# ChainSafe/lumenos

Measured on AMD Instinct MI355X. Metric: prove_eval_seconds_16384x4096, lower is better.
Workload: dtype u64; 1 GPU; Encode+Commit+InnerProduct(r,b)+QueryCols 16384x4096 LogN=14 L=12 K=2 rhoInv=2 queries=309; parallelism=1 GPU: the whole job resident in HBM

## Files before the change

lumenos_amd/csrc/lm_keyswitch.hip:

```cpp
#include <cstdlib>
#include <cstring>

#include "lm_ks_dev.h"

__host__ __device__ __forceinline__ size_t ks_ext_at(uint32_t b, uint32_t d, uint32_t t, uint32_t B, uint32_t beta) {
    return ((size_t)t * B + b) * beta + d;
}
__host__ __device__ __forceinline__ size_t ks_u_at(uint32_t pw, uint32_t t, uint32_t B, uint32_t L, uint32_t K) {
    return t < L ? (size_t)t * 2 * B + pw : (size_t)L * 2 * B + (size_t)pw * K + (t - L);
}
__host__ __device__ __forceinline__ size_t ks_key_at(uint32_t d, uint32_t w, uint32_t t, uint32_t beta) {
    return ((size_t)t * beta + d) * 2 + w;
}

static uint32_t ks_batch(const lumen_ctx *ctx) { return ctx->tune.ks_batch; }

__device__ __forceinline__ void mul128(u64 a, u64 b, u64 &lo, u64 &hi) {
    const u32 a0 = (u32)a, a1 = (u32)(a >> 32), b0 = (u32)b, b1 = (u32)(b >> 32);
    const u64 p0 = (u64)a0 * b0;
    const u64 p1 = lm_keep((u64)a0 * b1 + (p0 >> 32));
    const u64 p2 = lm_keep((u64)a1 * b0 + (u32)p1);
    hi = (u64)a1 * b1 + (p1 >> 32) + (p2 >> 32);
    lo = (p2 << 32) | (u32)p0;
}
// ... 67 lines not shown
        return;
    }
    const uint32_t d = blockIdx.x / B, b = blockIdx.x % B;
    const uint32_t l0 = 2 * d, l1 = l0 + 1;
    const u64 *c1 = acc + ((size_t)b * 2 + 1) * L * N;
    u64 *o0 = coef + ((size_t)b * L + l0) * N;
    const lm_qc q0 = lm_make_qc(mods.m[l0]);
    const tw_t s0 = yscale.t[l0];
    {
        const u64 *p = c1 + (size_t)l0 * N;
        auto ld = [&](uint32_t i0, u64 *v, int count) { lm_load_run(p, i0, v, count); };
        auto st = [&](uint32_t i, u64 v) { o0[i] = lm_shoup_cs(v, s0, q0.q, q0.nq); };
        lm_ntt_inverse<LOGN>(sm, tw_all + (size_t)l0 * N, q0, tid, nthreads, ld, st);
    }
    __syncthreads();
    {
        const lm_qc q1 = lm_make_qc(mods.m[l1]);
        const tw_t s1 = yscale.t[l1];
        const u64 *p = c1 + (size_t)l1 * N;
        u64 Ml, Mh;
        mul128(q0.q, q1.q, Ml, Mh);
        auto uni = [](u64 x) {
            return (u64)(uint32_t)__builtin_amdgcn_readfirstlane((int)(uint32_t)x) |
                   (u64)(uint32_t)__builtin_amdgcn_readfirstlane((int)(uint32_t)(x >> 32)) << 32;
        };
        const u128 M = ((u128)uni(Mh) << 64) | uni(Ml);
        auto ld = [&](uint32_t i0, u64 *v, int count) { lm_load_run(p, i0, v, count); };
        constexpr int R_LAST = lm_pass_r(LOGN, 0), LOG_T0 = LOGN - R_LAST;
        constexpr int PF = (1 << R_LAST) * 5 / 8;
        struct pack_t {
            u64 *o0;
            const lm_qc &q0, &q1;
            tw_t s1;
            u128 M;
            u64 y0[PF];
            __device__ __forceinline__ void pre(uint32_t w) {
#pragma unroll
                for (int k = 0; k < PF; k++) y0[k] = o0[w + ((uint32_t)k << LOG_T0)];
            }
            __device__ __forceinline__ void operator()(uint32_t i, u64 v, int k) {
                const u64 y1 = lm_shoup_cs(v, s1, q1.q, q1.nq);
                uint32_t j = i;
                asm volatile("" : "+v"(j));
                const u64 a = k < PF ? y0[k < PF ? k : 0] : o0[j];
                u64 hi, lo;
                pack_pair(a, y1, q0.q, q1.q, M, hi, lo);
                o0[j] = hi, o0[j + N] = lo;
                if (k >= PF && (k & 1)) asm volatile("" ::: "memory");
            }
        } st{o0, q0, q1, s1, M, {}};
        uint32_t tid1 = tid;
        asm volatile("" : "+v"(tid1));
        lm_ntt_inverse<LOGN>(sm, tw_all + (size_t)l1 * N, q1, tid1, nthreads, ld, st);
    }
}

struct pt_consts_t {
    u64 c[LM_MAX_LIMBS];
};
__global__ void k_pt_prepare(const u64 *__restrict__ pt, u64 *__restrict__ ptM, uint32_t logN, uint32_t nl,
                             lm_mods mods, pt_consts_t pc) {
    const size_t total = (size_t)nl << logN;
    for (size_t i = (size_t)blockIdx.x * blockDim.x + threadIdx.x; i < total; i += (size_t)gridDim.x * blockDim.x) {
        const uint32_t limb = (uint32_t)(i >> logN);
        u64 lo, hi;
        mul128(pt[i], pc.c[limb], lo, hi);
        ptM[i] = lm_mont_reduce(lo, hi, mods.m[limb].q, mods.m[limb].qneg);
    }
}
__global__ void k_mul_plain(const u64 *__restrict__ ct, u64 *__restrict__ out, const u64 *__restrict__ ptM,
                            size_t words, uint32_t logN, uint32_t nl, lm_mods mods) {
    const size_t stride = (size_t)gridDim.x * blockDim.x;
    const size_t N = (size_t)1 << logN;
    for (size_t i = (size_t)blockIdx.x * blockDim.x + threadIdx.x; i < words; i += stride) {
        const uint32_t limb = (uint32_t)((i >> logN) % nl);
        const size_t k = i & (N - 1);
        u64 lo, hi;
        mul128(ct[i], ptM[(size_t)limb * N + k], lo, hi);
        out[i] = lm_mont_reduce(lo, hi, mods.m[limb].q, mods.m[limb].qneg);
    }
}

template <int LOGN>
__global__ __launch_bounds__(lm_max_threads(LOGN)) void k_modup_ntt(const u64 *__restrict__ coef, const u64 *__restrict__ acc,
                                                    u64 *__restrict__ ext, const bx_t *__restrict__ bx,
                                                    uint32_t B, uint32_t L, uint32_t K, uint32_t beta,
                                                    const uint32_t *__restrict__ work, lm_mods mods,
                                                    const tw_t *__restrict__ tw_all) {
    extern __shared__ __attribute__((aligned(16))) u64 sm[];
    constexpr uint32_t N = 1u << LOGN;
    const uint32_t tid = threadIdx.x, nthreads = blockDim.x, LK = L + K;
    const uint32_t wk = work[blockIdx.x];
    const uint32_t b = wk & 0xFFFF, d = (wk >> 16) & 0xFF, t = wk >> 24;
    const bx_t c = bx[d * LK + t];
    u64 *o = ext + ks_ext_at(b, d, t, B, beta) * N;
    const lm_qc qc = lm_make_qc(mods.m[t]);
    const u64 *s0 = coef + ((size_t)b * L + d * K) * N;
    const u64 *s1 = c.ns == 2 ? s0 + N : s0;
    auto ld = [&](uint32_t i) { return bx_apply(c, s0[i], s1[i], qc); };
    lm_lds_runs st{sm};
    auto after = [&](uint32_t, uint32_t) {
        lm_linear_out<LOGN>(sm, tid, [&](uint32_t j, u64 v0, u64 v1) {
            ulonglong2 y;
            y.x = v0, y.y = v1;
            *reinterpret_cast<ulonglong2 *>(o + j) = y;
        });
    };
    lm_ntt_forward<LOGN>(sm, tw_all + (size_t)t * N, qc, tid, nthreads, ld, st, after);
}

#ifndef LM_MAC_COLS
#define LM_MAC_COLS 4
#endif
#ifndef LM_MAC_VEC
#define LM_MAC_VEC 1
#endif
#ifndef LM_MAC_PREFETCH
#define LM_MAC_PREFETCH 1
#endif
template <int VEC>
struct mac_vec;
template <>
struct mac_vec<1> {
    u64 v[1];
    static __device__ __forceinline__ mac_vec load(const u64 *p) { return mac_vec{{*p}}; }
    static __device__ __forceinline__ mac_vec load_once(const u64 *p) { return mac_vec{{__builtin_nontemporal_load(p)}}; }
    __device__ __forceinline__ void store(u64 *p) const { *p = v[0]; }
};
template <>
struct mac_vec<2> {
    u64 v[2];
    static __device__ __forceinline__ mac_vec load(const u64 *p) {
        const ulonglong2 a = *reinterpret_cast<const ulonglong2 *>(p);
        return mac_vec{{a.x, a.y}};
    }
    static __device__ __forceinline__ mac_vec load_once(const u64 *p) {
        return mac_vec{{__builtin_nontemporal_load(p), __builtin_nontemporal_load(p + 1)}};
    }
    __device__ __forceinline__ void store(u64 *p) const {
        ulonglong2 a;
        a.x = v[0], a.y = v[1];
        *reinterpret_cast<ulonglong2 *>(p) = a;
    }
};
struct mac_acc {
    u64 a0, a1, a3;
    u32 c0, c1;
    __device__ __forceinline__ void clear() { a0 = a1 = a3 = 0, c0 = c1 = 0; }
    __device__ __forceinline__ void value(u64 &lo, u64 &hi) const {
        lo = a0 + (a1 << 32);
        hi = a3 + c0 + (a1 >> 32) + ((u64)c1 << 32) + (lo < a0 ? 1 : 0);
    }
};
__device__ __forceinline__ void mac2(mac_acc &p, mac_acc &q, u64 x, u64 k0, u64 k1) {
    const u32 x0 = (u32)x, x1 = (u32)(x >> 32);
#if LM_ASM_SHOUP
    asm("v_mad_u64_u32 %[pa0], s[98:99], %[x0], %[k00], %[pa0]\n\t"
        "v_mad_u64_u32 %[qa0], s[90:91], %[x0], %[k10], %[qa0]\n\t"
        "v_mad_u64_u32 %[pa1], s[94:95], %[x0], %[k01], %[pa1]\n\t"
        "v_addc_co_u32_e64 %[pc0], s[96:97], %[pc0], 0, s[98:99]\n\t"
        "v_mad_u64_u32 %[qa1], s[92:93], %[x0], %[k11], %[qa1]\n\t"
        "v_addc_co_u32_e64 %[qc0], s[96:97], %[qc0], 0, s[90:91]\n\t"
        "v_mad_u64_u32 %[pa3], s[96:97], %[x1], %[k01], %[pa3]\n\t"
        "v_addc_co_u32_e64 %[pc1], s[96:97], %[pc1], 0, s[94:95]\n\t"
        "v_mad_u64_u32 %[pa1], s[98:99], %[x1], %[k00], %[pa1]\n\t"
        "v_addc_co_u32_e64 %[qc1], s[96:97], %[qc1], 0, s[92:93]\n\t"
        "v_mad_u64_u32 %[qa1], s[90:91], %[x1], %[k10], %[qa1]\n\t"
        "v_mad_u64_u32 %[qa3], s[96:97], %[x1], %[k11], %[qa3]\n\t"
        "v_addc_co_u32_e64 %[pc1], s[96:97], %[pc1], 0, s[98:99]\n\t"
        "v_addc_co_u32_e64 %[qc1], s[96:97], %[qc1], 0, s[90:91]"
        : [pa0] "+v"(p.a0), [pa1] "+v"(p.a1), [pa3] "+v"(p.a3), [pc0] "+v"(p.c0), [pc1] "+v"(p.c1),
          [qa0] "+v"(q.a0), [qa1] "+v"(q.a1), [qa3] "+v"(q.a3), [qc0] "+v"(q.c0), [qc1] "+v"(q.c1)
        : [x0] "v"(x0), [x1] "v"(x1), [k00] "v"((u32)k0), [k01] "v"((u32)(k0 >> 32)), [k10] "v"((u32)k1),
          [k11] "v"((u32)(k1 >> 32))
        : "s92", "s93", "s94", "s95", "s96", "s97", "s98", "s99", "s90", "s91");
#else
    auto one = [&](mac_acc &r, u64 k) {
        const u32 k0w = (u32)k, k1w = (u32)(k >> 32);
        u64 t = r.a0 + (u64)x0 * k0w;
        r.c0 += t < r.a0, r.a0 = t;
        t = r.a1 + (u64)x0 * k1w;
        r.c1 += t < r.a1, r.a1 = t;
        t = r.a1 + (u64)x1 * k0w;
        r.c1 += t < r.a1, r.a1 = t;
        r.a3 += (u64)x1 * k1w;
    };
    one(p, k0);
    one(q, k1);
#endif
}

// ... 372 lines not shown
    static const uint32_t v = [&] {
        hipDeviceProp_t prop;
        int per_cu = 0;
        if (hipGetDeviceProperties(&prop, ctx->device) != hipSuccess) return 256u;
        (void)hipFuncSetAttribute(reinterpret_cast<const void *>(&k_intt_pack<LOGN>),
                                  hipFuncAttributeMaxDynamicSharedMemorySize, 160 * 1024);
        if (hipOccupancyMaxActiveBlocksPerMultiprocessor(&per_cu, k_intt_pack<LOGN>, lm_nthreads(LOGN),
                                                         lm_lds_for(1u << LOGN)) != hipSuccess || per_cu < 1) {
            per_cu = (int)std::max<size_t>(1, std::min<size_t>(160 * 1024 / lm_lds_for(1u << LOGN), 2048 / lm_nthreads(LOGN)));
        }
        (void)hipGetLastError();
        if (ctx->tune.debug)
            fprintf(stderr, "[lumenos_hip] k_intt_pack<%d>: %d workgroup(s) per CU, %d CUs\n", LOGN, per_cu,
                    prop.multiProcessorCount);
        return (uint32_t)prop.multiProcessorCount * (uint32_t)per_cu;
    }();
    return v;
}
static uint32_t ks_fused_digits(lumen_ctx *ctx, uint32_t B, uint32_t L) {
    const long forced = ctx->tune.ks_fused_digits;
    const uint32_t pairs = L / 2;
    if (forced >= 0) return std::min<uint32_t>((uint32_t)forced, pairs);
    uint32_t slots = 0;
    switch (ctx->logN) {
#define LM_CASE(n) \
    case n: slots = intt_pack_slots<n>(ctx); break;
        LM_FOR_EACH_LOGN(LM_CASE)
#undef LM_CASE
    default: return 0;
    }
    for (uint32_t nf = pairs; nf >= 1; nf--)
        if (((uint64_t)B * nf) % slots == 0) return nf;
    return 0;
}

struct LaneGuard {
    lumen_ctx *ctx;
    hipStream_t saved;
    LaneGuard(lumen_ctx *c, int lane) : ctx(c), saved(c->stream) {
        if (lane) ctx->stream = ctx->stream2;
    }
    ~LaneGuard() { ctx->stream = saved; }
};

int rotate_accumulate(lumen_ctx *ctx, const u64 *acc, u64 *acc_out, uint32_t B, const lm_galois_key &gk,
                      KsTables *tb, const KsScratch &s) {
    const uint32_t N = ctx->N, L = ctx->L, K = ctx->K, LK = L + K, beta = tb->beta;
    const size_t lds = lm_fwd_lds(ctx->logN);
    const uint32_t threads = lm_fwd_threads(ctx->logN);
    const uint32_t nf = K == 2 ? ks_fused_digits(ctx, B, L) : 0;
    if (nf) {
        const size_t lds_i = lm_inv_lds(ctx->logN);
        const uint32_t grid = B * nf + B * (L - 2 * nf);
        lm_prof_scope ps(ctx, "ks_intt_c1", (uint64_t)B * L);
        switch (ctx->logN) {
#define LM_CASE(n)                                                                                              \
    case n:                                                                                                     \
        LM_LDS_ATTR(ctx, k_intt_pack<n>, lds_i);                                                                \
        hipLaunchKernelGGL(k_intt_pack<n>, dim3(grid), dim3(lm_inv_threads(ctx->logN)), lds_i, ctx->stream, acc, \
                           s.coef, B, L, nf, ctx->mods, tb->yscale, ctx->d_tw_inv);                             \
        break;
            LM_FOR_EACH_LOGN(LM_CASE)
#undef LM_CASE
        default:
            return lm_fail(ctx, "ring degree 2^%u has no kernel instantiation", ctx->logN);
        }
        LM_HIP(ctx, hipGetLastError());
    } else {
        if (int rc = lm_launch_ntt_strided(ctx, acc + (size_t)L * N, (size_t)2 * L * N, s.coef, (size_t)L * N, B,
                                           lm_map_q(L), true, "ks_intt_c1", &tb->yscale))
            return rc;
    }
    if (K == 2 && nf < beta) {
        lm_prof_scope ps(ctx, "ks_pack_v", (uint64_t)B);
        hipLaunchKernelGGL(k_pack_v, dim3(2048), dim3(256), 0, ctx->stream, s.coef + (size_t)2 * nf * N, (size_t)L * N,
                           B, beta - nf, K, 2 * nf, L - 2 * nf, ctx->logN, ctx->mods);
        LM_HIP(ctx, hipGetLastError());
    }
    {
        const uint64_t nb = (uint64_t)B * tb->pairs.size();
        const uint32_t *work = nullptr;
        if (int rc = modup_work_list(ctx, tb, B, &work)) return rc;
        lm_prof_scope ps(ctx, "ks_modup_ntt", nb);
        switch (ctx->logN) {
#define LM_CASE(n)                                                                                            \
    case n:                                                                                                   \
        LM_LDS_ATTR(ctx, k_modup_ntt<n>, lds);               \
        hipLaunchKernelGGL(k_modup_ntt<n>, dim3((uint32_t)nb), dim3(threads), lds, ctx->stream, s.coef, acc,  \
                           s.ext, tb->d_bx, B, L, K, beta, work, ctx->mods, ctx->d_tw_fwd);                   \
        break;
            LM_FOR_EACH_LOGN(LM_CASE)
#undef LM_CASE
        default:
            return lm_fail(ctx, "ring degree 2^%u has no kernel instantiation", ctx->logN);
        }
        LM_HIP(ctx, hipGetLastError());
    }
    {
        lm_prof_scope ps(ctx, "ks_mac", (uint64_t)B);
        dim3 grid(((N / LM_MAC_VEC + 255) / 256) * LK * ((B + LM_MAC_COLS - 1) / LM_MAC_COLS));
        hipLaunchKernelGGL(k_ks_mac, grid, dim3(256), 0, ctx->stream, s.ext, acc, gk.d_key, s.u, B, L, K, beta,
                           ctx->logN, ctx->mods);
        LM_HIP(ctx, hipGetLastError());
    }
    {
        lm_modmap mp;
        mp.period = K;
        for (uint32_t i = 0; i < LM_MAX_LIMBS; i++) mp.idx[i] = (uint8_t)(L + (i < K ? i : 0));
        u64 *up = s.u + ks_u_at(0, L, B, L, K) * N;
        const size_t pstride = (size_t)K * N;
        if (int rc = lm_launch_ntt_strided(ctx, up, pstride, up, pstride, B * 2, mp, true, "ks_intt_p", &tb->yscale))
            return rc;
        if (K == 2) {
            lm_prof_scope ps(ctx, "ks_pack_v", (uint64_t)B);
            hipLaunchKernelGGL(k_pack_v, dim3(2048), dim3(256), 0, ctx->stream, up, pstride, B * 2, 1u, K, L, K,
                               ctx->logN, ctx->mods);
            LM_HIP(ctx, hipGetLastError());
        }
    }
    {
        const uint32_t *work_down = nullptr;
        if (int rc = moddown_work_list(ctx, tb, B, &work_down)) return rc;
        lm_prof_scope ps(ctx, "ks_moddown_ntt", (uint64_t)B * 2 * L);
        switch (ctx->logN) {
#define LM_CASE(n)                                                                                            \
    case n:                                                                                                   \
        LM_LDS_ATTR(ctx, k_moddown_ntt<n>, lds);               \
        hipLaunchKernelGGL(k_moddown_ntt<n>, dim3(B * 2 * L), dim3(threads), lds, ctx->stream, s.u, acc,      \
                           acc_out, tb->d_bxp, tb->d_pinv, gk.d_index, gk.d_inv_index, work_down, B, L, K, ctx->mods, \
                           ctx->d_tw_fwd);                                                                    \
        break;
            LM_FOR_EACH_LOGN(LM_CASE)
#undef LM_CASE
        default:
            return lm_fail(ctx, "ring degree 2^%u has no kernel instantiation", ctx->logN);
        }
        LM_HIP(ctx, hipGetLastError());
    }
    return 0;
}

int get_scratch(lumen_ctx *ctx, uint32_t B, KsTables *tb, KsScratch *s, int lane = 0, u64 **group_acc = nullptr,
                size_t group_acc_bytes = 0) {
    const size_t N = ctx->N, L = ctx->L, LK = ctx->L + ctx->K, beta = tb->beta;
    const char *names[2][5] = {{"ks_coef", "ks_ext", "ks_u", "ks_acc2", "ks_acc"}, {"ks_coef_b", "ks_ext_b", "ks_u_b", "ks_acc2_b", "ks_acc"}};
    const int NB = group_acc ? 5 : 4;
    const size_t bytes[5] = {(size_t)B * L * N * 8, (size_t)B * beta * LK * N * 8, (size_t)B * 2 * LK * N * 8, (size_t)B * 2 * L * N * 8,
                             std::max(group_acc_bytes, (size_t)B * 2 * L * N * 8)};
    u64 *dummy = nullptr;
    u64 **slot[5] = {&s->coef, &s->ext, &s->u, &s->acc2, group_acc ? group_acc : &dummy};
    bool have = true;
    for (int c = 0; c < NB; c++) {
        auto it = ctx->scratch.find(names[lane][c]);
        have = have && it != ctx->scratch.end() && it->second.first && it->second.second >= bytes[c];
    }
    lm_galois_key gk;
    {
        LM_SHARED_LOCK(ctx);
        if (!ctx->gkeys.empty()) gk = ctx->gkeys.begin()->second;
    }
    const uint32_t Kc = ctx->tune.ks_placement;
    auto plain = [&]() -> int {
        bool ok = true;
        for (int c = 0; c < NB; c++) ok = (*slot[c] = (u64 *)lm_scratch(ctx, names[lane][c], bytes[c])) != nullptr && ok;
        return ok ? 0 : 1;
    };
    if (have || Kc < 2 || bytes[1] < ((size_t)64 << 20) || !gk.d_key) return plain();
    std::vector<void *> cand[5];
    bool fixed[5] = {false, false, false, false, false};
    for (int c = 0; c < NB; c++) {
        auto it = ctx->scratch.find(names[lane][c]);
// ... 401 lines not shown
```

lumenos_amd/csrc/lm_ntt.hip:

```cpp
#include "lm_ntt_dev.h"

template <int LOGN, bool INV>
__global__ __launch_bounds__(lm_max_threads(LOGN)) void k_limb_ntt(const u64 *src, size_t src_poly_stride, u64 *dst,
                                                   size_t dst_poly_stride, uint32_t npoly, lm_modmap map,
                                                   lm_mods mods, lm_ninv_t ninv,
                                                   const tw_t *__restrict__ tw_all) {
    extern __shared__ __attribute__((aligned(16))) u64 sm[];
    constexpr uint32_t N = 1u << LOGN;
    const uint32_t tid = threadIdx.x, nthreads = blockDim.x;
    const uint32_t limb = blockIdx.x / npoly, poly = blockIdx.x % npoly;
    const uint32_t mi = map.idx[limb];
    const lm_qc c = lm_make_qc(mods.m[mi]);
    const u64 *p = src + (size_t)poly * src_poly_stride + (size_t)limb * N;
    u64 *o = dst + (size_t)poly * dst_poly_stride + (size_t)limb * N;
    const tw_t *tw = tw_all + (size_t)mi * N;
    if (INV) {
        const tw_t ni = ninv.t[mi];
        auto st = [&](uint32_t i, u64 v) { o[i] = lm_shoup_cs(v, ni, c.q, c.nq); };
        auto ld = [&](uint32_t i0, u64 *v, int count) { lm_load_run(p, i0, v, count); };
        lm_ntt_inverse<LOGN>(sm, tw, c, tid, nthreads, ld, st);
    } else {
        auto ld = [&](uint32_t i) { return p[i]; };
        auto st = [&](uint32_t i0, const u64 *v, int count) {
            u64 r[8];
#pragma unroll
            for (int k = 0; k < 8; k++)
                if (k < count) r[k] = lm_reduce_s(v[k], c.q, c.nq, c.qinv64);
            lm_store_run(o, i0, r, count);
        };
        lm_ntt_forward<LOGN>(sm, tw, c, tid, nthreads, ld, st);
    }
}

int lm_launch_ntt_subring(lumen_ctx *ctx, uint32_t logn, const tw_t *tw, tw_t ninv_scale, const u64 *src,
                          size_t src_poly_stride, u64 *dst, size_t dst_poly_stride, uint32_t npoly,
                          uint32_t mod_idx, bool inverse, const mod_t *explicit_mod) {
    if (!npoly) return 0;
    lm_modmap map = lm_map_q(1);
    map.idx[0] = 0;
    lm_mods mods = ctx->mods;
    mods.m[0] = explicit_mod ? *explicit_mod : ctx->mods.m[mod_idx];
    lm_ninv_t ninv = lm_ninv_of(ctx);
    ninv.t[0] = ninv_scale;
    const size_t lds = inverse ? lm_inv_lds(logn) : lm_fwd_lds(logn);
    const uint32_t threads = inverse ? lm_inv_threads(logn) : lm_fwd_threads(logn);
    const dim3 grid(npoly), block(threads);
#define LM_LAUNCH(n)                                                                                          \
    case n:                                                                                                   \
        if (inverse) {                                                                                        \
            LM_LDS_ATTR(ctx, (k_limb_ntt<n, true>), lds);                                                     \
            hipLaunchKernelGGL((k_limb_ntt<n, true>), grid, block, lds, ctx->stream, src, src_poly_stride,    \
                               dst, dst_poly_stride, npoly, map, mods, ninv, tw);                             \
        } else {                                                                                              \
            LM_LDS_ATTR(ctx, (k_limb_ntt<n, false>), lds);                                                    \
            hipLaunchKernelGGL((k_limb_ntt<n, false>), grid, block, lds, ctx->stream, src, src_poly_stride,   \
                               dst, dst_poly_stride, npoly, map, mods, ninv, tw);                             \
        }                                                                                                     \
        break;
    switch (logn) {
        LM_FOR_EACH_LOGN(LM_LAUNCH)
    default:
        return lm_fail(ctx, "ring degree 2^%u has no kernel instantiation", logn);
    }
#undef LM_LAUNCH
    LM_HIP(ctx, hipGetLastError());
    return 0;
}

int lm_launch_ntt_strided(lumen_ctx *ctx, const u64 *src, size_t src_poly_stride, u64 *dst,
                          size_t dst_poly_stride, uint32_t npoly, const lm_modmap &map, bool inverse,
                          const char *prof_name, const lm_ninv_t *inv_scale) {
    if (!npoly || !map.period) return 0;
    const uint32_t N = ctx->N;
    const lm_ninv_t ninv = inv_scale ? *inv_scale : lm_ninv_of(ctx);
    const size_t lds = inverse ? lm_inv_lds(ctx->logN) : lm_fwd_lds(ctx->logN);
    const uint32_t threads = inverse ? lm_inv_threads(ctx->logN) : lm_fwd_threads(ctx->logN);
    (void)N;
    const uint64_t nblocks64 = (uint64_t)npoly * map.period;
    LM_CHECK(ctx, nblocks64 < (1ull << 31), "NTT grid too large: %llu", (unsigned long long)nblocks64);
    lm_prof_scope ps(ctx, prof_name ? prof_name : (inverse ? "limb_intt" : "limb_ntt"), nblocks64);
    const dim3 grid((uint32_t)nblocks64), block(threads);
#define LM_LAUNCH(n)                                                                                          \
    case n:                                                                                                   \
        if (inverse) {                                                                                        \
            LM_LDS_ATTR(ctx, (k_limb_ntt<n, true>), lds);           \
            hipLaunchKernelGGL((k_limb_ntt<n, true>), grid, block, lds, ctx->stream, src, src_poly_stride,    \
                               dst, dst_poly_stride, npoly, map, ctx->mods, ninv, ctx->d_tw_inv);             \
        } else {                                                                                              \
            LM_LDS_ATTR(ctx, (k_limb_ntt<n, false>), lds);           \
            hipLaunchKernelGGL((k_limb_ntt<n, false>), grid, block, lds, ctx->stream, src, src_poly_stride,   \
                               dst, dst_poly_stride, npoly, map, ctx->mods, ninv, ctx->d_tw_fwd);             \
        }                                                                                                     \
        break;
    switch (ctx->logN) {
        LM_FOR_EACH_LOGN(LM_LAUNCH)
    default:
        return lm_fail(ctx, "ring degree 2^%u has no kernel instantiation", ctx->logN);
    }
#undef LM_LAUNCH
    LM_HIP(ctx, hipGetLastError());
    return 0;
}

int lm_launch_ntt(lumen_ctx *ctx, u64 *d, uint32_t npoly, const lm_modmap &map, bool inverse) {
    const size_t stride = (size_t)map.period * ctx->N;
    return lm_launch_ntt_strided(ctx, d, stride, d, stride, npoly, map, inverse, nullptr, nullptr);
}

extern "C" int lumen_set_ntt(lumen_ctx *ctx, lumen_set *set, int inverse) {
    LM_CHECK(nullptr, ctx && set, "lumen_set_ntt: NULL argument");
    LM_ENTER(ctx);
    LM_FULL_WIDTH(ctx, set, "lumen_set_ntt");
    return lm_launch_ntt(ctx, set->d, set->count * 2, lm_map_q(set->nl), inverse != 0);
}
```

lumenos_amd/csrc/lm_ntt_dev.h:

```cpp
#pragma once
#include <cstring>
#include <type_traits>
#include <utility>

#include "lm_common.h"

#define LM_PAD(i) ((i) + ((i) >> 3))
template <int LOG_STRIDE>
__device__ __forceinline__ uint32_t lm_pad_at(uint32_t base, uint32_t pbase, int k) {
    if constexpr (LOG_STRIDE >= 3)
        return pbase + (uint32_t)k * ((1u << LOG_STRIDE) + (1u << (LOG_STRIDE - 3)));
    else
        return LM_PAD(base + ((uint32_t)k << LOG_STRIDE));
}
#define LM_MAX_PASSES 8

struct lm_ninv_t {
    tw_t t[LM_MAX_LIMBS];
};

__host__ __device__ constexpr int lm_ilog2(int x) { return x <= 1 ? 0 : 1 + lm_ilog2(x >> 1); }
#ifndef LM_COEFS_PER_LANE
#define LM_COEFS_PER_LANE 16
#endif
// ... 389 lines not shown
        lm_fwd_first<LOGN, R, cross>(sm, tw, c, tid, ld);
    else if constexpr (P == NP - 1)
        lm_fwd_last<LOGN, R>(sm, tw, c, tid, st);
    else
        lm_fwd_mid<LOGN, R, S0>(sm, tw, c, tid);
    if constexpr (P + 1 < NP) {
        if constexpr (P == 0 && cross)
            __syncthreads();
        else
            lm_wave_sync();
        lm_fwd_rec<LOGN, P + 1, S0 + R>(sm, tw, c, tid, ld, st);
    }
}
template <int LOGN>
__host__ __device__ constexpr int lm_fwd_run() {
    return 1 << lm_pass_r(LOGN, lm_npasses(LOGN) - 1);
}
struct lm_no_after {
    __device__ __forceinline__ void operator()(uint32_t, uint32_t) const {}
};

#ifndef LM_TW_XPASS
#define LM_TW_XPASS 1
#endif
template <int LOGN, int R, int S0, bool UW>
__device__ __forceinline__ void lm_fwd_mid_item(u64 *s, const lm_twset<R, UW> &T, const lm_qc &c, uint32_t w) {
    constexpr uint32_t log_tl = LOGN - S0 - R;
    const uint32_t blk = w >> log_tl, off = w & ((1u << log_tl) - 1);
    const uint32_t base = (blk << (log_tl + R)) + off;
    u64 e[1 << R];
    const uint32_t pb = LM_PAD(base);
#pragma unroll
    for (int k = 0; k < (1 << R); k++) e[k] = s[lm_pad_at<log_tl>(base, pb, k)];
    lm_fwd_stages<R, UW>(e, T, c);
#pragma unroll
    for (int k = 0; k < (1 << R); k++) s[lm_pad_at<log_tl>(base, pb, k)] = e[k];
}
template <class Loader, class Storer>
__device__ __forceinline__ void lm_fwd14_xpass(u64 *sm, const tw_t *tw, const lm_qc &c, uint32_t tid, Loader &ld,
                                               Storer &st) {
    constexpr int LOGN = 14;
    static_assert(lm_npasses(LOGN) == 4 && lm_pass_r(LOGN, 0) == 4 && lm_pass_r(LOGN, 1) == 4 &&
                      lm_pass_r(LOGN, 2) == 3 && lm_pass_r(LOGN, 3) == 3,
                  "written for the pass plan 4 | 4 3 3");
    using D4 = lm_deal<LOGN, 4>;
    using D3 = lm_deal<LOGN, 3>;
    static_assert(D4::reps == 1 && D3::reps == 2, "one item in pass 1, two in passes 2 and 3");
    lm_fwd_first<LOGN, 4, true>(sm, tw, c, tid, ld);
    lm_twset<4, true> T1;
    T1.load(tw, 4, D4::local(tid, 0) >> (LOGN - 8));
    __syncthreads();
    lm_twset<3, false> A, B;
    A.load(tw, 8, D3::local(tid, 0) >> (LOGN - 11));
    B.load(tw, 8, D3::local(tid, 1) >> (LOGN - 11));
    lm_fwd_mid_item<LOGN, 4, 4, true>(sm, T1, c, D4::local(tid, 0));
    lm_wave_sync();
    lm_fwd_mid_item<LOGN, 3, 8, false>(sm, A, c, D3::local(tid, 0));
    A.load(tw, 11, D3::local(tid, 0));
    lm_fwd_mid_item<LOGN, 3, 8, false>(sm, B, c, D3::local(tid, 1));
    B.load(tw, 11, D3::local(tid, 1));
    lm_wave_sync();
#pragma unroll
    for (uint32_t m = 0; m < 2; m++) {
        const uint32_t base = D3::local(tid, m) << 3;
        u64 e[8];
#pragma unroll
        for (int k = 0; k < 8; k++) e[k] = sm[LM_PAD(base + k)];
        lm_fwd_stages<3, false>(e, m ? B : A, c);
        st(base, e, 8);
    }
}

template <int LOGN, bool XPASS = true, class Loader, class Storer, class After = lm_no_after>
__device__ __forceinline__ void lm_ntt_forward(u64 *sm, const tw_t *tw, const lm_qc &c, uint32_t tid, uint32_t,
                                               Loader &ld, Storer &st, After after = After()) {
    static_assert(lm_npasses(LOGN) >= 2, "a transform needs a loading and a storing pass");
    if constexpr (LOGN == 14 && XPASS && LM_TW_XPASS && LM_COEFS_PER_LANE == 16 && !lm_has_pre<Storer>::value)
        lm_fwd14_xpass(sm, tw, c, tid, ld, st);
    else
        lm_fwd_rec<LOGN, 0, 0>(sm, tw, c, tid, ld, st);
    after(0u, 1u << LOGN);
}

template <int LOGN, int R, class Loader>
__device__ __forceinline__ void lm_inv_first(u64 *s, const tw_t *tw, const lm_qc &c, uint32_t tid, Loader &ld) {
    using D = lm_deal<LOGN, R>;
    if (!D::valid(tid)) return;
#pragma unroll 1
    for (uint32_t m = 0; m < D::reps; m++) {
        const uint32_t w = D::local(tid, m);
        const uint32_t base = w << R;
        u64 e[1 << R];
        lm_inv_twset<R, false, true> T;
        T.load(tw, LOGN, 0, w);
        ld(base, e, 1 << R);
        lm_inv_stages<R, false, false, true>(e, T, c);
#pragma unroll
        for (int k = 0; k < (1 << R); k++) s[LM_PAD(base + k)] = e[k];
    }
}

#ifndef LM_INV_TW_PREFETCH
#define LM_INV_TW_PREFETCH 1
#endif
template <int LOGN, int R, int LT>
__device__ __forceinline__ void lm_inv_mid(u64 *s, const tw_t *tw, const lm_qc &c, uint32_t tid) {
    using D = lm_deal<LOGN, R>;
    if (!D::valid(tid)) return;
    constexpr bool UW = LT >= 6;
    lm_inv_twset<R, UW, false> T[2];
    T[0].load(tw, LOGN, LT, D::local(tid, 0) >> LT);
#pragma unroll
    for (uint32_t m = 0; m < D::reps; m++) {
        const uint32_t w = D::local(tid, m);
        const uint32_t blk = w >> LT, off = w & ((1u << LT) - 1);
        const uint32_t base = (blk << (LT + R)) + off;
        u64 e[1 << R];
        const uint32_t pb = LM_PAD(base);
#pragma unroll
        for (int k = 0; k < (1 << R); k++) e[k] = s[lm_pad_at<LT>(base, pb, k)];
        if (LM_INV_TW_PREFETCH && m + 1 < D::reps) T[(m + 1) & 1].load(tw, LOGN, LT, D::local(tid, m + 1) >> LT);
        if (!LM_INV_TW_PREFETCH && m) T[0].load(tw, LOGN, LT, blk);
        lm_inv_stages<R, UW, false, false>(e, T[LM_INV_TW_PREFETCH ? (m & 1) : 0], c);
#pragma unroll
        for (int k = 0; k < (1 << R); k++) s[lm_pad_at<LT>(base, pb, k)] = e[k];
    }
}

template <class S, class = void>
struct lm_has_slot : std::false_type {};
template <class S>
struct lm_has_slot<S, std::void_t<decltype(std::declval<S &>()(0u, (u64)0, 0))>> : std::true_type {};

template <int LOGN, int R, class Storer>
__device__ __forceinline__ void lm_inv_last(const u64 *s, const tw_t *tw, const lm_qc &c, uint32_t tid, Storer &st) {
    constexpr uint32_t log_t0 = LOGN - R, items = 1u << log_t0, NT = lm_nthreads(LOGN);
    constexpr uint32_t reps = items / NT ? items / NT : 1;
    lm_inv_twset<R, true, false> T;
    T.load(tw, LOGN, log_t0, 0);
#pragma unroll 1
    for (uint32_t m = 0; m < reps; m++) {
        const uint32_t w = tid + m * NT;
        if (items < NT && w >= items) break;
        u64 e[1 << R];
#pragma unroll
        for (int k = 0; k < (1 << R); k++) e[k] = s[lm_pad_at<log_t0>(w, LM_PAD(w), k)];
        if constexpr (lm_has_pre<Storer>::value) st.pre(w);
        lm_inv_stages<R, true, true, false>(e, T, c);
#pragma unroll
        for (int k = 0; k < (1 << R); k++) {
            if constexpr (lm_has_slot<Storer>::value)
                st(w + ((uint32_t)k << log_t0), e[k], k);
            else
                st(w + ((uint32_t)k << log_t0), e[k]);
        }
    }
}

template <int LOGN, int P, int LT, class Loader, class Storer>
__device__ __forceinline__ void lm_inv_rec(u64 *sm, const tw_t *tw, const lm_qc &c, uint32_t tid, Loader &ld,
                                           Storer &st) {
    constexpr int NP = lm_npasses(LOGN), R = lm_pass_r(LOGN, NP - 1 - P);
    constexpr bool cross = lm_cross_r(LOGN) > 0;
    if constexpr (P == 0)
        lm_inv_first<LOGN, R>(sm, tw, c, tid, ld);
    else if constexpr (P == NP - 1)
// ... 63 lines not shown
```

Before: 1.800 s.

## Add wave-local 512-thread forward NTT for logN=14 with half-size LDS

After: 1.742 s, median of 6. -3.2%, faster.

```diff
diff --git a/lumenos_amd/csrc/lm_keyswitch.hip b/lumenos_amd/csrc/lm_keyswitch.hip
--- a/lumenos_amd/csrc/lm_keyswitch.hip
+++ b/lumenos_amd/csrc/lm_keyswitch.hip
@@ -173,7 +173,7 @@
 }
 
 template <int LOGN>
-__global__ __launch_bounds__(lm_max_threads(LOGN)) void k_modup_ntt(const u64 *__restrict__ coef, const u64 *__restrict__ acc,
+__global__ __launch_bounds__(lm_fwdw_threads(LOGN), lm_fwdw_waves(LOGN)) void k_modup_ntt(const u64 *__restrict__ coef, const u64 *__restrict__ acc,
                                                     u64 *__restrict__ ext, const bx_t *__restrict__ bx,
                                                     uint32_t B, uint32_t L, uint32_t K, uint32_t beta,
                                                     const uint32_t *__restrict__ work, lm_mods mods,
@@ -189,15 +189,21 @@
     const u64 *s0 = coef + ((size_t)b * L + d * K) * N;
     const u64 *s1 = c.ns == 2 ? s0 + N : s0;
     auto ld = [&](uint32_t i) { return bx_apply(c, s0[i], s1[i], qc); };
-    lm_lds_runs st{sm};
-    auto after = [&](uint32_t, uint32_t) {
-        lm_linear_out<LOGN>(sm, tid, [&](uint32_t j, u64 v0, u64 v1) {
-            ulonglong2 y;
-            y.x = v0, y.y = v1;
-            *reinterpret_cast<ulonglong2 *>(o + j) = y;
-        });
+    auto out = [&](uint32_t j, u64 v0, u64 v1) {
+        ulonglong2 y;
+        y.x = v0, y.y = v1;
+        *reinterpret_cast<ulonglong2 *>(o + j) = y;
     };
-    lm_ntt_forward<LOGN>(sm, tw_all + (size_t)t * N, qc, tid, nthreads, ld, st, after);
+    if constexpr (LOGN == 14) {
+        (void)nthreads;
+        lm_w14_runs st{sm};
+        auto after = [&](uint32_t i0, uint32_t) { lm_w14_linear_out(sm, tid, i0, out); };
+        lm_ntt_forward_w14(sm, tw_all + (size_t)t * N, qc, tid, ld, st, after);
+    } else {
+        lm_lds_runs st{sm};
+        auto after = [&](uint32_t, uint32_t) { lm_linear_out<LOGN>(sm, tid, out); };
+        lm_ntt_forward<LOGN>(sm, tw_all + (size_t)t * N, qc, tid, nthreads, ld, st, after);
+    }
 }
 
 #ifndef LM_MAC_COLS
@@ -736,11 +742,12 @@
         const uint32_t *work = nullptr;
         if (int rc = modup_work_list(ctx, tb, B, &work)) return rc;
         lm_prof_scope ps(ctx, "ks_modup_ntt", nb);
+        const lm_geom gm = lm_fwdw_geom(ctx->logN);
         switch (ctx->logN) {
 #define LM_CASE(n)                                                                                            \
     case n:                                                                                                   \
-        LM_LDS_ATTR(ctx, k_modup_ntt<n>, lds);               \
-        hipLaunchKernelGGL(k_modup_ntt<n>, dim3((uint32_t)nb), dim3(threads), lds, ctx->stream, s.coef, acc,  \
+        LM_LDS_ATTR(ctx, k_modup_ntt<n>, gm.lds);                                                             \
+        hipLaunchKernelGGL(k_modup_ntt<n>, dim3((uint32_t)nb), dim3(gm.threads), gm.lds, ctx->stream, s.coef, acc, \
                            s.ext, tb->d_bx, B, L, K, beta, work, ctx->mods, ctx->d_tw_fwd);                   \
         break;
             LM_FOR_EACH_LOGN(LM_CASE)
diff --git a/lumenos_amd/csrc/lm_ntt.hip b/lumenos_amd/csrc/lm_ntt.hip
--- a/lumenos_amd/csrc/lm_ntt.hip
+++ b/lumenos_amd/csrc/lm_ntt.hip
@@ -1,7 +1,9 @@
 #include "lm_ntt_dev.h"
 
+__host__ __device__ constexpr int lm_limb_ntt_threads(int logN, bool inv) { return inv ? lm_max_threads(logN) : lm_fwdw_threads(logN); }
+__host__ __device__ constexpr int lm_limb_ntt_waves(int logN, bool inv) { return inv ? 1 : lm_fwdw_waves(logN); }
 template <int LOGN, bool INV>
-__global__ __launch_bounds__(lm_max_threads(LOGN)) void k_limb_ntt(const u64 *src, size_t src_poly_stride, u64 *dst,
+__global__ __launch_bounds__(lm_limb_ntt_threads(LOGN, INV), lm_limb_ntt_waves(LOGN, INV)) void k_limb_ntt(const u64 *src, size_t src_poly_stride, u64 *dst,
                                                    size_t dst_poly_stride, uint32_t npoly, lm_modmap map,
                                                    lm_mods mods, lm_ninv_t ninv,
                                                    const tw_t *__restrict__ tw_all) {
@@ -28,7 +30,10 @@
                 if (k < count) r[k] = lm_reduce_s(v[k], c.q, c.nq, c.qinv64);
             lm_store_run(o, i0, r, count);
         };
-        lm_ntt_forward<LOGN>(sm, tw, c, tid, nthreads, ld, st);
+        if constexpr (LOGN == 14)
+            lm_ntt_forward_w14(sm, tw, c, tid, ld, st);
+        else
+            lm_ntt_forward<LOGN>(sm, tw, c, tid, nthreads, ld, st);
     }
 }
 
@@ -42,8 +47,8 @@
     mods.m[0] = explicit_mod ? *explicit_mod : ctx->mods.m[mod_idx];
     lm_ninv_t ninv = lm_ninv_of(ctx);
     ninv.t[0] = ninv_scale;
-    const size_t lds = inverse ? lm_inv_lds(logn) : lm_fwd_lds(logn);
-    const uint32_t threads = inverse ? lm_inv_threads(logn) : lm_fwd_threads(logn);
+    const size_t lds = inverse ? lm_inv_lds(logn) : lm_fwdw_geom(logn).lds;
+    const uint32_t threads = inverse ? lm_inv_threads(logn) : lm_fwdw_geom(logn).threads;
     const dim3 grid(npoly), block(threads);
 #define LM_LAUNCH(n)                                                                                          \
     case n:                                                                                                   \
@@ -73,8 +78,8 @@
     if (!npoly || !map.period) return 0;
     const uint32_t N = ctx->N;
     const lm_ninv_t ninv = inv_scale ? *inv_scale : lm_ninv_of(ctx);
-    const size_t lds = inverse ? lm_inv_lds(ctx->logN) : lm_fwd_lds(ctx->logN);
-    const uint32_t threads = inverse ? lm_inv_threads(ctx->logN) : lm_fwd_threads(ctx->logN);
+    const size_t lds = inverse ? lm_inv_lds(ctx->logN) : lm_fwdw_geom(ctx->logN).lds;
+    const uint32_t threads = inverse ? lm_inv_threads(ctx->logN) : lm_fwdw_geom(ctx->logN).threads;
     (void)N;
     const uint64_t nblocks64 = (uint64_t)npoly * map.period;
     LM_CHECK(ctx, nblocks64 < (1ull << 31), "NTT grid too large: %llu", (unsigned long long)nblocks64);
diff --git a/lumenos_amd/csrc/lm_ntt_dev.h b/lumenos_amd/csrc/lm_ntt_dev.h
--- a/lumenos_amd/csrc/lm_ntt_dev.h
+++ b/lumenos_amd/csrc/lm_ntt_dev.h
@@ -495,6 +495,168 @@
     after(0u, 1u << LOGN);
 }
 
+#define LM_W14_THREADS 512
+#ifndef LM_W14_SCHED_FENCE
+#define LM_W14_SCHED_FENCE 1
+#endif
+#if LM_W14_SCHED_FENCE
+#define LM_W14_FENCE() __builtin_amdgcn_sched_barrier(0)
+#else
+#define LM_W14_FENCE() ((void)0)
+#endif
+#ifndef LM_W14_PF3
+#define LM_W14_PF3 0
+#endif
+#ifndef LM_W14_PF4
+#define LM_W14_PF4 0
+#endif
+struct lm_w14_plan {
+    static constexpr int R1 = 5, R2 = 3, R3 = 3, R4 = 3;
+};
+static_assert(lm_w14_plan::R1 + lm_w14_plan::R2 + lm_w14_plan::R3 + lm_w14_plan::R4 == 14, "the four passes cover the 14 stages once");
+static_assert((1 << lm_w14_plan::R1) == 32 && (1 << lm_w14_plan::R2) * 4 == 32 && (1 << lm_w14_plan::R3) * 4 == 32 &&
+                  (1 << lm_w14_plan::R4) * 4 == 32,
+              "pass 1 is one item of 32 coefficients per lane, passes 2-4 four items of 8");
+static_assert(LM_W14_THREADS * 32 == 1 << 14 && LM_W14_THREADS / 64 == 8, "8 waves x 64 lanes x 32 coefficients");
+__device__ __forceinline__ uint32_t lm_w14_pos(uint32_t i) { return LM_PAD(((i >> 11) << 10) | (i & 1023u)); }
+__device__ __forceinline__ uint32_t lm_w14_at(uint32_t pbase, uint32_t k) { return pbase + k + (k >> 3); }
+
+template <int R>
+__device__ __forceinline__ void lm_fwd_stages_first(u64 *e, const tw_t *tw, const lm_qc &c) {
+#pragma unroll
+    for (int st = 0; st < R; st++) {
+        const int span = (1 << R) >> st, half = span >> 1, CH = half < 8 ? half : 8;
+#pragma unroll
+        for (int g = 0; g < (1 << st); g++) {
+            const tw_t W = lm_tw_load<true>(tw, (1u << st) + g);
+#pragma unroll
+            for (int k0 = 0; k0 < half; k0 += CH) {
+                u64 sum[CH];
+#pragma unroll
+                for (int k = 0; k < CH; k++)
+                    sum[k] = lm_shoup3<true>(e[g * span + k0 + k + half], W.w, W.wp, c.nq, e[g * span + k0 + k]);
+#pragma unroll
+                for (int k = 0; k < CH; k++) {
+                    u64 &x = e[g * span + k0 + k];
+                    e[g * span + k0 + k + half] = lm_bfly_diff(x, c.q3, sum[k]);
+                    x = sum[k];
+                }
+            }
+        }
+    }
+}
+
+template <class Loader, class Storer, class After = lm_no_after>
+__device__ __forceinline__ void lm_ntt_forward_w14(u64 *sm, const tw_t *tw, const lm_qc &c, uint32_t tid, Loader &ld,
+                                                   Storer &st, After after = After()) {
+    const uint32_t w = tid >> 6, l = tid & 63;
+    u64 e[32];
+#pragma unroll
+    for (int r = 0; r < 32; r++) e[r] = ld(((uint32_t)r << 9) | tid);
+    lm_fwd_stages_first<5>(e, tw, c);
+    const uint32_t p1 = LM_PAD(tid), p2 = LM_PAD((w << 10) | l);
+    lm_twset<3, true> T2[2];
+    T2[0].load(tw, 5, (w << 2) | 0);
+    u64 e0[16];
+#pragma unroll
+    for (int h = 0; h < 2; h++) {
+#pragma unroll
+        for (int r = 0; r < 32; r++)
+            if (((r >> 1) & 1) == h) sm[lm_w14_at(p1, (uint32_t)((r >> 2) << 10 | (r & 1) << 9))] = e[r];
+        __syncthreads();
+#pragma unroll
+        for (int r = 0; r < 16; r++) (h ? e[16 + r] : e0[r]) = sm[lm_w14_at(p2, (uint32_t)r << 6)];
+        if (h == 0) __syncthreads();
+    }
+#pragma unroll
+    for (int r = 0; r < 16; r++) e[r] = e0[r];
+#pragma unroll
+    for (int gq = 0; gq < 4; gq++) {
+        if (gq + 1 < 4) T2[(gq + 1) & 1].load(tw, 5, (w << 2) | (uint32_t)(gq + 1));
+        lm_fwd_stages<3, true>(e + 8 * gq, T2[gq & 1], c);
+    }
+    const uint32_t p3 = LM_PAD((w << 10) | ((l >> 3) << 6) | (l & 7));
+    lm_twset<3, false> T3[2];
+    T3[0].load(tw, 8, (w << 5) | (l >> 3));
+#pragma unroll
+    for (int h = 0; h < 2; h++) {
+        lm_wave_sync();
+#pragma unroll
+        for (int r = 16 * h; r < 16 * h + 16; r++) sm[lm_w14_at(p2, (uint32_t)(r & 15) << 6)] = e[r];
+        lm_wave_sync();
+#pragma unroll
+        for (int r = 16 * h; r < 16 * h + 16; r++)
+            e[r] = sm[lm_w14_at(p3, (uint32_t)(((r >> 3) & 1) << 9 | (r & 7) << 3))];
+    }
+#pragma unroll
+    for (int m = 0; m < 4; m++) {
+        LM_W14_FENCE();
+        if (LM_W14_PF3 && m + 1 < 4) T3[(m + 1) & 1].load(tw, 8, (w << 5) | ((uint32_t)(m + 1) << 3) | (l >> 3));
+        if (!LM_W14_PF3 && m) T3[0].load(tw, 8, (w << 5) | ((uint32_t)m << 3) | (l >> 3));
+        lm_fwd_stages<3, false>(e + 8 * m, T3[LM_W14_PF3 ? (m & 1) : 0], c);
+    }
+    const uint32_t p4 = LM_PAD((w << 10) | (l << 3));
+    lm_twset<3, false> T4[2];
+    T4[0].load(tw, 11, (w << 8) | l);
+#pragma unroll
+    for (int h = 0; h < 2; h++) {
+        lm_wave_sync();
+#pragma unroll
+        for (int r = 16 * h; r < 16 * h + 16; r++)
+            sm[lm_w14_at(p3, (uint32_t)(((r >> 3) & 1) << 9 | (r & 7) << 3))] = e[r];
+        lm_wave_sync();
+#pragma unroll
+        for (int r = 16 * h; r < 16 * h + 16; r++)
+            e[r] = sm[lm_w14_at(p4, (uint32_t)(((r >> 3) & 1) << 9 | (r & 7)))];
+    }
+    constexpr bool TWPF = LM_W14_PF4 && !lm_has_pre<Storer>::value;
+    lm_wave_sync();
+#pragma unroll
+    for (int m = 0; m < 4; m++) {
+        LM_W14_FENCE();
+        const uint32_t i0 = (w << 11) | ((uint32_t)m << 9) | (l << 3);
+        if constexpr (lm_has_pre<Storer>::value) st.pre(i0);
+        if (TWPF && m + 1 < 4) T4[(m + 1) & 1].load(tw, 11, (w << 8) | ((uint32_t)(m + 1) << 6) | l);
+        if (!TWPF && m) T4[0].load(tw, 11, (w << 8) | ((uint32_t)m << 6) | l);
+        lm_fwd_stages<3, false>(e + 8 * m, T4[TWPF ? (m & 1) : 0], c);
+        st(i0, e + 8 * m, 8);
+        if (m & 1) {
+            lm_wave_sync();
+            after((uint32_t)(m >> 1) << 10, 1024u);
+            lm_wave_sync();
+        }
+    }
+}
+struct lm_w14_runs {
+    u64 *sm;
+    __device__ __forceinline__ void operator()(uint32_t i0, const u64 *v, int count) const {
+        const uint32_t pb = lm_w14_pos(i0);
+#pragma unroll
+        for (int k = 0; k < 8; k++)
+            if (k < count) sm[pb + k] = v[k];
+    }
+};
+template <class F>
+__device__ __forceinline__ void lm_w14_linear_out(const u64 *sm, uint32_t tid, uint32_t i0, F f) {
+    const uint32_t w = tid >> 6, lane = tid & 63;
+    const uint32_t pb = LM_PAD((w << 10) | (2 * lane));
+#pragma unroll
+    for (uint32_t k = 0; k < 8; k++) {
+        const uint32_t j = (w << 11) | i0 | (2 * lane + 128 * k);
+        f(j, sm[lm_w14_at(pb, 128 * k)], sm[lm_w14_at(pb, 128 * k) + 1]);
+    }
+}
+
+__host__ __device__ constexpr int lm_fwdw_threads(int logN) { return logN == 14 ? LM_W14_THREADS : lm_nthreads(logN); }
+__host__ __device__ constexpr int lm_fwdw_waves(int logN) { return logN == 14 ? 4 : 1; }
+struct lm_geom {
+    uint32_t threads;
+    size_t lds;
+};
+static inline lm_geom lm_fwdw_geom(uint32_t logN) {
+    return logN == 14 ? lm_geom{(uint32_t)LM_W14_THREADS, lm_lds_for(1u << 13)} : lm_geom{lm_fwd_threads(logN), lm_fwd_lds(logN)};
+}
+
 template <int LOGN, int R, class Loader>
 __device__ __forceinline__ void lm_inv_first(u64 *s, const tw_t *tw, const lm_qc &c, uint32_t tid, Loader &ld) {
     using D = lm_deal<LOGN, R>;
```
